# StanfordASL/GuSTO.jl

Measured on AMD Instinct MI355X. Metric: converged trajectories/sec (batched SCP), freeflyer_se2 N=50, inputs resident in HBM, higher is better.
Workload: dtype f64

## Files before the change

### gusto.jl_amd/csrc/common.hpp

```cpp
#pragma once
#include <hip/hip_runtime.h>
#include <math.h>
#include <stdint.h>

#include "gusto_hip.h"

namespace gusto {

#define GD __device__ __forceinline__
typedef double v4d __attribute__((ext_vector_type(4)));

constexpr int ROW_HARD = 0;
constexpr int ROW_PEN = 1;
constexpr int ROW_PEN_TR = 2;
constexpr int ROW_PEN_EQ = 3;
constexpr int ROW_HARD_EQ = 4;
constexpr int ROW_EQ = 5;
GD bool row_is_hard(int kind) { return kind == ROW_HARD || kind == ROW_HARD_EQ; }

constexpr int RS_T = 0, RS_LAM = 1, RS_LAMB = 2, RS_S = 3, RS_DT = 4, RS_DL = 5, RS_DS = 6, RS_KA = 7, RS_KB = 8,
              RS_NVAR = 9;

#ifndef GUSTO_DUBINS_WAVES
#define GUSTO_DUBINS_WAVES 2
#endif
#ifndef GUSTO_WAVES_PER_EU
#define GUSTO_WAVES_PER_EU 1
#endif

#ifndef GUSTO_TO_SWEEP_CALL
#define GUSTO_TO_SWEEP_CALL true
#endif
#ifndef GUSTO_TO4_SWEEP_CALL
#define GUSTO_TO4_SWEEP_CALL true
#endif
#ifndef GUSTO_SWEEP_DPP
#define GUSTO_SWEEP_DPP 1
#endif
#ifndef GUSTO_FACTOR_LDS
#define GUSTO_FACTOR_LDS 1
#endif
#ifndef GUSTO_FACTOR_LDS_MV
#define GUSTO_FACTOR_LDS_MV 1
#endif
#ifndef GUSTO_FACTOR_LDS_HUU
#define GUSTO_FACTOR_LDS_HUU 0
#endif
#ifndef GUSTO_FACTOR_LDS_ROWS
#define GUSTO_FACTOR_LDS_ROWS 1
#endif
#ifndef GUSTO_USE_MFMA
#define GUSTO_USE_MFMA true
#endif
constexpr int GUSTO_TO_FREEFLYER_SE2 = 4, GUSTO_TO_ASTROBEE_SE3 = 5, GUSTO_TO_ASTROBEE_SE3_MANIFOLD = 6;
constexpr double TRAJOPT_DEFECT_REG = 1e-4;
constexpr int RS_EARLIER = 0, RS_ROW = 1, RS_ROW_LANE = 2;
template <int MODEL> struct MT;
template <> struct MT<GUSTO_FREEFLYER_SE2> {
    static constexpr int NDEF = 0;
    static constexpr int n = 6, m = 3, WS = 2, NFIX = 3, NHU = 2;
    static constexpr int WAVES_PER_EU = GUSTO_WAVES_PER_EU;
    static constexpr int RS_FORM = RS_ROW;
    static constexpr bool SWEEP_CALL = false;
    static constexpr bool SWEEP_DPP = GUSTO_SWEEP_DPP;
    static constexpr bool FACTOR_LDS = GUSTO_FACTOR_LDS;
    static constexpr bool MFMA = false;
    static constexpr int SCHED_PROBE = 2;
    static constexpr int SCHED_SLICE = 4;
    static constexpr bool LTI = true, HAS_OBS = true;
    static constexpr bool PG2 = true;
    static constexpr int pg_r0(int c) { return c < 3 ? c : (c < 6 ? c - 3 : c - 6); }
    static constexpr int pg_r1(int c) { return c < 3 ? c + 3 : (c < 6 ? c : c - 3); }
    static constexpr bool Anz(int i, int j) { return j == i + 3; }
    static constexpr bool Mnz(int i, int j) { return i == j || j == i + 3; }
    static constexpr bool Bnz(int i, int j) { return i == j + 3; }
    static constexpr bool Gnz(int i, int j) { return i == j || i == j + 3; }
    static constexpr bool Hnz(int, int) { return true; }
};
template <> struct MT<GUSTO_DUBINS_CAR> {
    static constexpr int NDEF = 0;
    static constexpr int n = 3, m = 1, WS = 2, NFIX = 6, NHU = 2;
    static constexpr int WAVES_PER_EU = GUSTO_DUBINS_WAVES;
    static constexpr int RS_FORM = RS_ROW;
    static constexpr bool SWEEP_CALL = false;
    static constexpr bool SWEEP_DPP = false;
    static constexpr bool FACTOR_LDS = false;
    static constexpr bool MFMA = false;
    static constexpr int SCHED_PROBE = 1; static constexpr int SCHED_SLICE = 0;
    static constexpr bool LTI = false, HAS_OBS = false;
    static constexpr bool PG2 = false;
    static constexpr int pg_r0(int) { return 0; }
    static constexpr int pg_r1(int) { return 0; }
    static constexpr bool Anz(int, int) { return true; }
    static constexpr bool Mnz(int, int) { return true; }
    static constexpr bool Bnz(int, int) { return true; }
    static constexpr bool Gnz(int, int) { return true; }
    static constexpr bool Hnz(int, int) { return true; }
};
template <> struct MT<GUSTO_ASTROBEE_SE3> {
    static constexpr int NDEF = 0;
    static constexpr int n = 12, m = 6, WS = 3, NFIX = 3, NHU = 2;
    static constexpr int WAVES_PER_EU = 1;
    static constexpr int RS_FORM = RS_ROW_LANE;
    static constexpr bool SWEEP_CALL = true;
    static constexpr bool SWEEP_DPP = false;
    static constexpr bool FACTOR_LDS = false;
    static constexpr bool MFMA = GUSTO_USE_MFMA;
    static constexpr int SCHED_PROBE = 1; static constexpr int SCHED_SLICE = 0;
    static constexpr bool LTI = false, HAS_OBS = true;
    static constexpr bool PG2 = false;
    static constexpr int pg_r0(int) { return 0; }
    static constexpr int pg_r1(int) { return 0; }
    static constexpr bool Anz(int i, int j) { return i < 3 ? j == i + 3 : (i < 6 ? false : (i < 9 ? j >= 6 : j >= 9)); }
    static constexpr bool Mnz(int i, int j) { return i < 3 ? (j == i || j == i + 3) : (i < 6 ? j == i : (i < 9 ? j >= 6 : j >= 9)); }
    static constexpr bool Bnz(int i, int j) { return j < 3 ? i == j + 3 : i == j + 6; }
    static constexpr bool Gnz(int i, int j) { return j < 3 ? (i == j || i == j + 3) : i >= 6; }
    static constexpr bool Hnz(int i, int j) { return i / 3 == j / 3; }
};
template <> struct MT<GUSTO_ASTROBEE_SE3_MANIFOLD> {
    static constexpr int NDEF = 0;
    static constexpr int n = 13, m = 6, WS = 3, NFIX = 5, NHU = 2;
    static constexpr int WAVES_PER_EU = 1;
    static constexpr int RS_FORM = RS_EARLIER;
    static constexpr bool SWEEP_CALL = true ;
    static constexpr bool SWEEP_DPP = false;
    static constexpr bool FACTOR_LDS = false;
    static constexpr bool MFMA = GUSTO_USE_MFMA;
    static constexpr int SCHED_PROBE = 1; static constexpr int SCHED_SLICE = 0;
    static constexpr bool LTI = false, HAS_OBS = true;
    static constexpr bool PG2 = false;
    static constexpr int pg_r0(int) { return 0; }
    static constexpr int pg_r1(int) { return 0; }
    static constexpr bool Anz(int i, int j) { return i < 3 ? j == i + 3 : (i < 6 ? false : (i < 10 ? j >= 6 : j >= 10)); }
    static constexpr bool Mnz(int i, int j) { return i < 3 ? (j == i || j == i + 3) : (i < 6 ? j == i : (i < 10 ? j >= 6 : j >= 10)); }
    static constexpr bool Bnz(int i, int j) { return j < 3 ? i == j + 3 : i == j + 7; }
    static constexpr bool Gnz(int i, int j) { return j < 3 ? (i == j || i == j + 3) : i >= 6; }
    static constexpr int hblk(int i) { return i < 3 ? 0 : (i < 6 ? 1 : (i < 10 ? 2 : 3)); }
    static constexpr bool Hnz(int i, int j) { return hblk(i) == hblk(j); }
};

template <> struct MT<GUSTO_TO_FREEFLYER_SE2> {
    using G = MT<GUSTO_FREEFLYER_SE2>;
    static constexpr int NDEF = 6, n = 6, m = 3 + NDEF, WS = 2, NFIX = 3, NHU = 2 + 2 * NDEF;
    static constexpr int WAVES_PER_EU = 1, SCHED_PROBE = 0, SCHED_SLICE = 0;
    static constexpr int RS_FORM = RS_ROW;
    static constexpr bool SWEEP_DPP = false;
    static constexpr bool FACTOR_LDS = false;
    static constexpr bool SWEEP_CALL = GUSTO_TO4_SWEEP_CALL, MFMA = false, LTI = false, HAS_OBS = true, PG2 = false;
    static constexpr int pg_r0(int) { return 0; }
    static constexpr int pg_r1(int) { return 0; }
    static constexpr bool Anz(int i, int j) { return G::Anz(i, j); }
    static constexpr bool Mnz(int i, int j) { return G::Mnz(i, j); }
    static constexpr bool Bnz(int i, int j) { return j < G::m && G::Bnz(i, j); }
    static constexpr bool Gnz(int i, int j) { return j < G::m ? G::Gnz(i, j) : i == j - G::m; }
    static constexpr bool Hnz(int, int) { return true; }
};
template <> struct MT<GUSTO_TO_ASTROBEE_SE3> {
    using G = MT<GUSTO_ASTROBEE_SE3>;
    static constexpr int NDEF = 12, n = 12, m = 6 + NDEF, WS = 3, NFIX = 3, NHU = 2 + 2 * NDEF;
    static constexpr int WAVES_PER_EU = 1, SCHED_PROBE = 0, SCHED_SLICE = 0;
    static constexpr int RS_FORM = RS_ROW;
    static constexpr bool SWEEP_DPP = false;
    static constexpr bool FACTOR_LDS = false;
    static constexpr bool SWEEP_CALL = GUSTO_TO_SWEEP_CALL, MFMA = false, LTI = false, HAS_OBS = true, PG2 = false;
    static constexpr int pg_r0(int) { return 0; }
    static constexpr int pg_r1(int) { return 0; }
    static constexpr bool Anz(int i, int j) { return G::Anz(i, j); }
    static constexpr bool Mnz(int i, int j) { return G::Mnz(i, j); }
    static constexpr bool Bnz(int i, int j) { return j < G::m && G::Bnz(i, j); }
    static constexpr bool Gnz(int i, int j) { return j < G::m ? G::Gnz(i, j) : i == j - G::m; }
    static constexpr bool Hnz(int, int) { return true; }
};

template <> struct MT<GUSTO_TO_ASTROBEE_SE3_MANIFOLD> {
    using G = MT<GUSTO_ASTROBEE_SE3_MANIFOLD>;
    static constexpr int NDEF = 13, n = 13, m = 6 + NDEF, WS = 3, NFIX = 5, NHU = 2 + 2 * NDEF;
    static constexpr int WAVES_PER_EU = 1, SCHED_PROBE = 0, SCHED_SLICE = 0;
    static constexpr int RS_FORM = RS_ROW;
    static constexpr bool SWEEP_DPP = false;
    static constexpr bool FACTOR_LDS = false;
    static constexpr bool SWEEP_CALL = GUSTO_TO_SWEEP_CALL, MFMA = false, LTI = false, HAS_OBS = true, PG2 = false;
    static constexpr int pg_r0(int) { return 0; }
    static constexpr int pg_r1(int) { return 0; }
    static constexpr bool Anz(int i, int j) { return G::Anz(i, j); }
    static constexpr bool Mnz(int i, int j) { return G::Mnz(i, j); }
    static constexpr bool Bnz(int i, int j) { return j < G::m && G::Bnz(i, j); }
    static constexpr bool Gnz(int i, int j) { return j < G::m ? G::Gnz(i, j) : i == j - G::m; }
    static constexpr bool Hnz(int, int) { return true; }
};
constexpr double TRAJOPT_EQ_DELTA = 1e-8;

inline void warm_defaults(int model, gusto_ipm_opts& io) {
    if (io.mu_floor < 0) io.mu_floor = (model == GUSTO_ASTROBEE_SE3_MANIFOLD) ? 1e-10 : 1e-11;
    if (io.sigma_max < 0) io.sigma_max = (model == GUSTO_TO_FREEFLYER_SE2 || model == GUSTO_TO_ASTROBEE_SE3 || model == GUSTO_TO_ASTROBEE_SE3_MANIFOLD) ? 0.0 : 0.1;
    if (!(io.mu_warm < 0)) { if (io.mu_warm_gain < 0) io.mu_warm_gain = 0.0; return; }
    switch (model) {
    case GUSTO_DUBINS_CAR: io.mu_warm = 1e-9; io.mu_warm_gain = 0.0; io.mu_warm_max = 1e-9; break;
    case GUSTO_FREEFLYER_SE2: io.mu_warm = 1e-4; io.mu_warm_gain = 0.1; io.mu_warm_max = 1e-2; break;
    case GUSTO_ASTROBEE_SE3: io.mu_warm = 1e-6; io.mu_warm_gain = 1.0; io.mu_warm_max = 1e-2; break;
    default: io.mu_warm = 1e-4; io.mu_warm_gain = 1.0; io.mu_warm_max = 1e-2; break;
    }
}
constexpr double IPM_DIVERGED = 1e3;
GD double warm_mu(const gusto_ipm_opts& io, double c) {
    if (io.mu_warm == 0.0) return 0.0;
    return fmin(fmax(io.mu_warm, io.mu_warm_max), fmax(io.mu_warm, io.mu_warm_gain * c * c));
}

GD constexpr int sidx(int i, int j, int n) {
    return i <= j ? i * n - i * (i - 1) / 2 + (j - i) : j * n - j * (j - 1) / 2 + (i - j);
}

template <int MODEL> struct Rec {
    using T = MT<MODEL>;
    static constexpr int n = T::n, m = T::m, NZ = n + m;
    static constexpr int r64(int c) { return (c + 63) / 64 * 64; }
    static constexpr bool S_TRI = false;
    static constexpr int NS = S_TRI ? m * (m + 1) / 2 : m * m;
    static constexpr int SQQ = r64(NZ * (NZ + 1) / 2), SNN = r64(n * n + 1), SKD = r64(2 * m * n + NS + 1);
    static constexpr int oK = 0, oD = m * n, oS = 2 * m * n;
    static constexpr int KD_DUMMY = 2 * m * n + NS;
    static constexpr int sS(int i, int l) {
        if (!S_TRI) return oS + i * m + l;
        const int a = i < l ? i : l, b = i < l ? l : i;
        return oS + a * m - a * (a - 1) / 2 + (b - a);
    }
};

template <int MODEL> struct SpPG {
    using T = MT<MODEL>;
    static constexpr int n = T::n, m = T::m;
    static constexpr int pos_phi(int l, int i) {
        int c = 0;
// ... 384 lines not shown
GD double rcp_nr(double d) {
    double r = __builtin_amdgcn_rcp(d);
    double e = fma(-d, r, 1.0);
    r = fma(r, e, r);
    e = fma(-d, r, 1.0);
    r = fma(r, e, r);
    return r;
}

GD double rsqrt_nr(double d) {
    double r = __builtin_amdgcn_rsq(d);
    const double h = 0.5 * d;
    r = r * (1.5 - h * r * r);
    r = r * (1.5 - h * r * r);
    return r;
}

template <int m> GD bool chol_inv(const double* S, double* Li) {
    double L[m][m], r[m];
    bool ok = true;
#pragma unroll
    for (int i = 0; i < m; i++)
#pragma unroll
        for (int j = 0; j < m; j++) { L[i][j] = 0; Li[i * m + j] = 0; }
#pragma unroll
    for (int j = 0; j < m; j++) {
        double d = S[j * m + j];
#pragma unroll
        for (int l = 0; l < j; l++) d -= L[j][l] * L[j][l];
        if (!(d > 0.0)) ok = false;
        r[j] = rsqrt_nr(d);
        L[j][j] = d * r[j];
#pragma unroll
        for (int i = j + 1; i < m; i++) {
            double s = S[i * m + j];
#pragma unroll
            for (int l = 0; l < j; l++) s -= L[i][l] * L[j][l];
            L[i][j] = s * r[j];
        }
    }
#pragma unroll
    for (int j = 0; j < m; j++) {
        Li[j * m + j] = r[j];
#pragma unroll
        for (int i = j + 1; i < m; i++) {
            double s = 0;
#pragma unroll
            for (int l = j; l < i; l++) s -= L[i][l] * Li[l * m + j];
            Li[i * m + j] = s * r[i];
        }
    }
    return ok;
}

GD bool inv_spd_rt(const double* S, double* Sinv, double* Lw, int n) {
    bool ok = true;
    for (int i = 0; i < n * n; i++) { Lw[i] = 0; Sinv[i] = 0; }
    for (int j = 0; j < n; j++) {
        double d = S[j * n + j];
        for (int l = 0; l < j; l++) d -= Lw[j * n + l] * Lw[j * n + l];
        if (!(d > 0.0)) ok = false;
        d = sqrt(d);
        Lw[j * n + j] = d;
        for (int i = j + 1; i < n; i++) {
            double s = S[i * n + j];
            for (int l = 0; l < j; l++) s -= Lw[i * n + l] * Lw[j * n + l];
            Lw[i * n + j] = s / d;
        }
    }
    for (int j = 0; j < n; j++) {
        Sinv[j * n + j] = 1.0 / Lw[j * n + j];
        for (int i = j + 1; i < n; i++) {
            double s = 0;
            for (int l = j; l < i; l++) s -= Lw[i * n + l] * Sinv[l * n + j];
            Sinv[i * n + j] = s / Lw[i * n + i];
        }
    }
    for (int i = 0; i < n; i++)
        for (int j = 0; j < n; j++) {
            double s = 0;
            for (int l = (i > j ? i : j); l < n; l++) s += Sinv[l * n + i] * Sinv[l * n + j];
            Lw[i * n + j] = s;
        }
    for (int i = 0; i < n * n; i++) Sinv[i] = Lw[i];
    return ok;
}

}
```

### gusto.jl_amd/csrc/factor1w.hpp

```cpp
#pragma once

namespace gusto {


template <int MODEL, class BLK> GD double* pg_buf(const BLK& K, int k) {
    using T = MT<MODEL>;
    using R = Rec<MODEL>;
    constexpr int NPG = T::n * (T::n + T::m);
    if constexpr (LdsC<MODEL, true>::PG_LDS) return K.pgl + k * NPG;
    else if constexpr (T::LTI) return K.sPG + (k == 0 ? 2 * NPG : 0);
    else return K.sPG + (k & 1) * NPG;
}

template <int MODEL> GD void factor_sweep_1w(SweepView<MODEL> K, double* fail, Prof& pf) {
    using T = MT<MODEL>;
    using R = Rec<MODEL>;
    using C = LdsC<MODEL, true>;
    constexpr int n = T::n, m = T::m, NZ = n + m, NQ = NZ * (NZ + 1) / 2, NPG = n * NZ, NN = n * n, NZN = NZ * n;
    constexpr int RT = (NPG + 63) / 64, RQ = (NQ + 63) / 64, RN = (NN + 63) / 64, RZ = (NZN + 63) / 64, RKD = R::SKD / 64;
    const int tid = K.tid, N = K.N;
    int zJ[RZ], zG[RZ], hI[RQ], hJ[RQ], nI[RN], nJ[RN], tL[RT], tC[RT];
#pragma unroll
    for (int r = 0; r < RT; r++) { const int e = tid + 64 * r; tL[r] = (e < NPG) ? e / NZ : 0; tC[r] = (e < NPG) ? e % NZ : 0; }
#pragma unroll
// ... 359 lines not shown
                if (tid == 0) {
#pragma unroll
                    for (int e = 0; e < m * (m + 1) / 2; e++) K.kdl[k * C::KDS + 2 * m * n + e] = sp[e];
                }
            } else {
                double sv[RKD];
#pragma unroll
                for (int r = 0; r < RKD; r++) sv[r] = 0;
#pragma unroll
                for (int a = 0; a < m; a++)
#pragma unroll
                    for (int c = 0; c <= a; c++) {
                        double s = 0;
#pragma unroll
                        for (int l = a; l < m; l++) s += Li[l * m + a] * Li[l * m + c];
#pragma unroll
                        for (int r = 0; r < RKD; r++) {
                            if (64 * r + 63 < R::oS || 64 * r >= R::oS + m * m) continue;
                            const int e = tid + 64 * r - R::oS;
                            sv[r] = (e == a * m + c || e == c * m + a) ? s : sv[r];
                        }
                    }
#pragma unroll
                for (int r = 0; r < RKD; r++) {
                    const int e = tid + 64 * r;
                    double v = (r < RN) ? kdv[r < RN ? r : 0] : 0.0;
                    if (64 * r + 63 >= R::oS && 64 * r < R::oS + m * m) { if (e >= R::oS) v = sv[r]; }
                    K.KD[(size_t)k * R::SKD + e] = v;
                }
            }
        }
        if (!T::LTI && !C::PG_LDS && k > 0) {
#pragma unroll
            for (int r = 0; r < RT; r++) { const int e = tid + 64 * r; if (e < NPG) K.sPG[((k - 1) & 1) * NPG + e] = pgn[r]; }
        }
        pf.tick(PF_F7);
        K.sync();
        pf.tick(PF_FCD);
    }
}

template <int MODEL> GD void factor_sweep_pg2(SweepView<MODEL> K, double* fail, Prof& pf) {
    using T = MT<MODEL>;
    using R = Rec<MODEL>;
    using C = LdsC<MODEL, true>;
    constexpr int n = T::n, m = T::m, NZ = n + m, NQ = NZ * (NZ + 1) / 2, NPG = n * NZ, NN = n * n, NZN = NZ * n, h3 = n / 2,
                  NH = n * (n + 1) / 2;
    static_assert(T::PG2 && T::LTI && C::KD_LDS && NQ <= 64 && NZN <= 64 && NN <= 64 && n >= 2 * m, "shape");
    static_assert(T::pg_r1(0) == T::pg_r0(0) + h3 && T::pg_r1(n) == T::pg_r0(n) + h3 && T::pg_r1(n - 1) == T::pg_r0(n - 1) + h3, "PG2 row pairs");
    static_assert(NH + NN < R::SNN && !C::BIG, "P | Pi record, dummy slot");
    constexpr bool F_MV = T::FACTOR_LDS && GUSTO_FACTOR_LDS_MV, F_HUU = T::FACTOR_LDS && GUSTO_FACTOR_LDS_HUU,
                   F_ROWS = T::FACTOR_LDS && GUSTO_FACTOR_LDS_ROWS;
    static_assert(!(F_MV || F_HUU || F_ROWS) || (n == 6 && m == 3), "FACTOR_LDS: rows of three 128-bit reads, m = 2 + 1");
    constexpr bool PG_UPPER = [] { for (int c = 0; c < NZ; c++) if (!(T::pg_r0(c) < h3 && T::pg_r1(c) == T::pg_r0(c) + h3)) return false; return true; }();
    static_assert(!F_MV || PG_UPPER, "F_MV: pg_r0(c) < n/2 and pg_r1(c) = pg_r0(c) + n/2 for every column of [Phi Gam]");
    const int tid = K.tid, N = K.N;
    const int ijh = K.lut[tid < NQ ? tid : 0], hc = ijh >> 8, hj = ijh & 255, i0 = T::pg_r0(hc), j0 = T::pg_r0(hj);
    const int zc = tid < NZN ? tid / n : 0, zg = tid < NZN ? tid % n : 0, z0 = T::pg_r0(zc);
    const int ri = tid < n ? tid : 0;
    const bool isnu = tid >= 8 && tid < 8 + n;
    const bool on = tid < NN;
    const int i = on ? tid / n : 0, j = on ? tid % n : 0;
    const LPtr<double> L = K.lds;
    typedef double v2d __attribute__((ext_vector_type(2)));
    auto ld2 = [&](int off) { return *(const __attribute__((address_space(3))) v2d*)(L.p + off); };
    const int dmy = C::sT0 + (tid & 15);
    static_assert(n * NZ >= 16 + 36, "dummy slot");
    constexpr int oHuu = C::sT0 + 46, NHU = m * (m + 1) / 2;
    static_assert(oHuu % 2 == 0 && 15 + (2 * m - 1) * n < 46 && 15 + NHU < 46 && 46 + NHU <= n * NZ, "H_uu behind the dummy slots, in the T buffer");
    constexpr int NZH = F_ROWS ? NZ + 1 : NZ, oZu = (C::sZ + 1) & ~1;
    static_assert(!F_ROWS || (C::sHh % 2 == 0 && NZH % 2 == 0 && n * NZH <= NZ * NZ && oZu + 4 * n <= C::sZ + NZN), "128-bit rows of H_yu and Z_u");
    auto pcol = [](int j_) { return 2 * (j_ % h3) + j_ / h3; };
    static_assert(C::sP % 2 == 0 && C::sPi % 2 == 0 && n % 2 == 0 && C::vecs % 2 == 0, "16-byte aligned rows");
    const int oPP = C::sP + i0 * n + 2 * j0, oPZ = C::sPi + zg * n + (F_MV ? 2 * z0 : z0), oPr = C::sP + ri * n, oPir = C::sPi + ri * n;
    const int oRow = tid < n ? C::sP + tid * n : (isnu ? C::sPi + (tid - 8) * n : C::sP);
    const int wH1 = tid < NQ ? ((hc >= n && F_HUU) ? oHuu + sidx(hc - n, hj - n, m) : ((hc >= n && F_ROWS) ? dmy : C::sHh + hc * NZH + hj))
                             : dmy;
    const int wZ = tid < NZN ? (F_ROWS ? (zc >= n ? oZu + zg * 4 + (zc - n) : dmy) : C::sZ + tid) : dmy;
    const int oHi = C::sHh + i * NZH + n, oHj = C::sHh + j * NZH + n, oPn = C::sHh + (i < j ? i : j) * NZH + (i < j ? j : i);
    const int oZi = F_ROWS ? oZu + i * 4 : C::sZ + n * n + i, oZj = F_ROWS ? oZu + j * 4 : C::sZ + n * n + j;
    const int wP = on ? C::sP + i * n + pcol(j) : dmy, wPi = on ? C::sPi + j * n + (F_MV ? pcol(i) : i) : dmy, wGd = on ? C::sGd + tid : dmy;
    const int vecs = C::vecs, oCv = vecs + 3 * N * n, oRv = vecs + 4 * N * n, oNun = vecs + 6 * N * n;
    const int wRv = tid < n ? oRv + tid : dmy, wNun = tid < n ? oNun + tid : dmy, sRv = tid < n ? n : 0;
    const int wRN = tid < n ? oRv + tid : (isnu ? oNun + (tid - 8) : dmy), sRN = (tid < n || isnu) ? n : 0;
    const int kdo = K.kd_off;
    const int wKD = tid < n ? kdo + tid : dmy, sKD = tid < n ? C::KDS : 0;
    const int wSi = tid == 0 ? kdo + 2 * m * n : dmy, sSi = tid == 0 ? C::KDS : 0;
    const int ep = (on && i <= j) ? sidx(i, j, n) : R::SNN - 1, eq = on ? NH + tid : R::SNN - 1;
    struct PGC { double a0, a1, b0, b1, zv0, zv1; };
    double Bd[n * m];
    Dyn<MODEL>::B(*K.mpp, Bd);
    auto pg_main = [&](int r_, int c_) { return K.PGk(N - 1)[r_ * NZ + c_]; };
    auto pg_zero = [&](int r_, int c_) {
        double v = 0.0;
#pragma unroll
        for (int q = 0; q < n * m; q++) if (c_ >= n && q == r_ * m + (c_ - n)) v = 0.5 * K.dt * Bd[q];
        return v;
    };
    PGC cN, c0;
    cN.a0 = pg_main(i0, hc); cN.a1 = pg_main(i0 + h3, hc); cN.b0 = pg_main(j0, hj); cN.b1 = pg_main(j0 + h3, hj);
    cN.zv0 = pg_main(z0, zc); cN.zv1 = pg_main(z0 + h3, zc);
    c0.a0 = pg_zero(i0, hc); c0.a1 = pg_zero(i0 + h3, hc); c0.b0 = pg_zero(j0, hj); c0.b1 = pg_zero(j0 + h3, hj);
    c0.zv0 = pg_zero(z0, zc); c0.zv1 = pg_zero(z0 + h3, zc);
    const double eterm = pg_main(zg, zc) + ((zc == zg) ? 1.0 : 0.0);
    const bool egoal = K.is_goal(zg);
    L[wP] = 0.0; L[wPi] = 0.0; L[wZ] = 0.0;
    double gdR = 0.0, zR = 0.0;
    if (tid < R::SNN) K.Paft[(size_t)(N - 1) * R::SNN + tid] = 0.0;
    double qq = K.kdl[(N - 1) * C::KDS + (tid < NQ ? tid : 0)];
    double LiP[m * m], wiP[m];
#pragma unroll
    for (int e = 0; e < m * m; e++) LiP[e] = 0.0;
#pragma unroll
    for (int e = 0; e < m; e++) wiP[e] = 0.0;
    bool okall = true;
    K.sync();

    auto tail = [&](int kt, const double* zi, const double* zj) {
        double pin = zR, gd = gdR;
        double vi[m], vj[m], dj[m];
#pragma unroll
        for (int a = 0; a < m; a++) {
            double s3 = 0, s4 = 0;
#pragma unroll
            for (int l = 0; l <= a; l++) { s3 += LiP[a * m + l] * zi[l]; s4 += LiP[a * m + l] * zj[l]; }
            vi[a] = s3; vj[a] = s4;
        }
#pragma unroll
        for (int a = 0; a < m; a++) {
            double s2 = 0;
#pragma unroll
            for (int l = a; l < m; l++) s2 += LiP[l * m + a] * vj[l];
            dj[a] = s2;
        }
#pragma unroll
        for (int l = 0; l < m; l++) { pin -= wiP[l] * vj[l]; gd += vi[l] * vj[l]; }
        L[wPi] = pin; gdR = gd;
        K.Paft[(size_t)(kt - 1) * R::SNN + eq] = pin;
#pragma unroll
        for (int a = 0; a < m; a++) L[wKD + kt * sKD + (m + a) * n] = dj[a];
    };

    auto msync = [&]() {
#ifdef GUSTO_STRICT_SYNC
        asm volatile("s_waitcnt vmcnt(0) lgkmcnt(0)\n\ts_barrier" ::: "memory");
#endif
        __builtin_amdgcn_fence(__ATOMIC_ACQ_REL, "wavefront");
    };
#if defined(GUSTO_PROFILE) && defined(GUSTO_STAGE_PROF)
#define STAMP(v) const unsigned long long v = __builtin_amdgcn_s_memtime()
#define STAMPS_END() do { pf.acc[PF_FPRE] += (long long)(t1_ - t0_); pf.acc[PF_FAB] += (long long)(t2_ - t1_); \
                          pf.acc[PF_F4] += (long long)(t3_ - t2_); pf.acc[PF_F5] += (long long)(t4_ - t3_); pf.acc[PF_FCD] += (long long)(t5_ - t4_); } while (0)
#else
#define STAMP(v) do {} while (0)
#define STAMPS_END() do {} while (0)
#endif
    auto ld3 = [&](int oi, int oj, double* vi, double* vj) {
        const v2d a2 = ld2(oi), b2 = ld2(oj);
        vi[0] = a2.x; vi[1] = a2.y; vi[2] = L[oi + 2]; vj[0] = b2.x; vj[1] = b2.y; vj[2] = L[oj + 2];
    };
    auto stage = [&](int k, const PGC& c, bool last) {
        STAMP(t0_);
        const v2d pA = ld2(oPP), pB = ld2(oPP + h3 * n);
        const double p00 = pA.x, p01 = pA.y, p10 = pB.x, p11 = pB.y;
        double ra[n], rb[n];
        if constexpr (!F_MV) {
#pragma unroll
            for (int l = 0; l < n; l += 2) {
                const v2d a2 = ld2(oPr + l), b2 = ld2(oCv + k * n + l);
                ra[l / 2] = a2.x; ra[l / 2 + h3] = a2.y; rb[l] = b2.x; rb[l + 1] = b2.y;
            }
        }
        double zi[m], zj[m];
        if constexpr (F_ROWS) ld3(oZi, oZj, zi, zj);
        else {
#pragma unroll
            for (int l = 0; l < m; l++) { zi[l] = L[oZi + l * n]; zj[l] = L[oZj + l * n]; }
        }
        const double qqn = K.kdl[((k > 0) ? k - 1 : 0) * C::KDS + (tid < NQ ? tid : 0)];
        const double h = qq + c.a0 * (c.b0 * p00 + c.b1 * p01) + c.a1 * (c.b0 * p10 + c.b1 * p11);
        L[wH1] = h;
        if constexpr (!F_MV) {
            double rr = 0;
#pragma unroll
            for (int l = 0; l < n; l++) rr += ra[l] * rb[l];
            L[wRv + k * sRv] = rr;
        }
        STAMP(t1_);
        msync();
        double S[m * m], Li[m * m];
        if constexpr (F_HUU) {
            const v2d s0 = ld2(oHuu), s1 = ld2(oHuu + 2), s2 = ld2(oHuu + 4);
            const double su[NHU] = {s0.x, s0.y, s1.x, s1.y, s2.x, s2.y};
#pragma unroll
            for (int a = 0; a < m; a++)
#pragma unroll
                for (int b = 0; b < m; b++) S[a * m + b] = su[sidx(a, b, m)];
        } else {
#pragma unroll
            for (int a = 0; a < m; a++)
#pragma unroll
                for (int b = 0; b < m; b++) {
                    const int e = sidx(n + (a < b ? a : b), n + (a < b ? b : a), NZ);
                    S[a * m + b] = readlane_f64(h, e);
                }
        }
        double hi[m], hjv[m];
        if constexpr (F_ROWS) ld3(oHi, oHj, hi, hjv);
        else {
#pragma unroll
            for (int l = 0; l < m; l++) { hi[l] = L[oHi + l]; hjv[l] = L[oHj + l]; }
        }
        double pn = L[oPn];
        tail(k + 1 < N ? k + 1 : N - 1, zi, zj);
        STAMP(t2_);
        msync();
        const double zb0 = F_MV ? ld2(oPZ).x : L[oPZ], zb1 = F_MV ? ld2(oPZ).y : L[oPZ + h3];
        double pa[n];
#pragma unroll
        for (int l = 0; l < n; l += 2) {
            const v2d a2 = ld2((F_MV ? oRow : oPir) + l);
            if constexpr (F_MV) {
                const v2d b2 = ld2(oCv + k * n + l);
                pa[l / 2] = a2.x; pa[l / 2 + h3] = a2.y; rb[l] = b2.x; rb[l + 1] = b2.y;
            } else { pa[l] = a2.x; pa[l + 1] = a2.y; }
        }
        okall = chol_inv<m>(S, Li) && okall;
        STAMP(t3_);
        {
            double z = c.zv0 * zb0 + c.zv1 * zb1;
            const double zE = fma(0.5, eterm, z);
            z = (last && egoal) ? zE : z;
            L[wZ] = z;
            zR = z;
            double rr = 0;
#pragma unroll
            for (int l = 0; l < n; l++) rr += pa[l] * rb[l];
            if constexpr (F_MV) L[wRN + k * sRN] = rr;
            else L[wNun + k * sRv] = rr;
        }
        STAMP(t4_);
        double wi[m], wj[m], kj[m];
#pragma unroll
        for (int a = 0; a < m; a++) {
            double s1 = 0, s2 = 0;
#pragma unroll
            for (int l = 0; l <= a; l++) { s1 += Li[a * m + l] * hi[l]; s2 += Li[a * m + l] * hjv[l]; }
            wi[a] = s1; wj[a] = s2;
        }
#pragma unroll
        for (int a = 0; a < m; a++) {
            double s1 = 0;
#pragma unroll
            for (int l = a; l < m; l++) s1 += Li[l * m + a] * wj[l];
            kj[a] = s1;
        }
#pragma unroll
        for (int l = 0; l < m; l++) pn -= wi[l] * wj[l];
        L[wP] = pn;
        K.Paft[(size_t)(k - 1) * R::SNN + ep] = pn;
#pragma unroll
        for (int a = 0; a < m; a++) L[wKD + k * sKD + a * n] = kj[a];
        {
#pragma unroll
            for (int a = 0; a < m; a++)
#pragma unroll
                for (int b = 0; b <= a; b++) {
                    double s1 = 0;
#pragma unroll
                    for (int l = a; l < m; l++) s1 += Li[l * m + a] * Li[l * m + b];
                    L[wSi + k * sSi + sidx(b, a, m)] = s1;
                }
        }
        qq = qqn;
#pragma unroll
        for (int e = 0; e < m * m; e++) LiP[e] = Li[e];
#pragma unroll
        for (int e = 0; e < m; e++) wiP[e] = wi[e];
        msync();
        STAMP(t5_);
        STAMPS_END();
    };
#undef STAMP
#undef STAMPS_END

    for (int k = N - 1; k >= 1; k--) stage(k, cN, k == N - 1);
    stage(0, c0, false);
    {
        double zi[m], zj[m];
        if constexpr (F_ROWS) ld3(oZi, oZj, zi, zj);
        else {
#pragma unroll
            for (int l = 0; l < m; l++) { zi[l] = L[oZi + l * n]; zj[l] = L[oZj + l * n]; }
        }
        tail(0, zi, zj);
    }
    L[wGd] = gdR;
    if (!okall) *fail = 1.0;
    K.sync();
    (void)pf;
}

#ifndef GUSTO_COSTATE_ADJOINT
#define GUSTO_COSTATE_ADJOINT 1
#endif
template <int MODEL> constexpr bool costate_adjoint() { return GUSTO_COSTATE_ADJOINT && MT<MODEL>::SWEEP_CALL && MT<MODEL>::MFMA; }
#ifndef GUSTO_ADJ_MAX_IT
#define GUSTO_ADJ_MAX_IT 20
#endif
#ifndef GUSTO_ADJ_ACC
#define GUSTO_ADJ_ACC 3
#endif
constexpr int ADJ_FLAG = 9;
template <int MODEL> GD bool costate_adjoint_now() { return gusto_dyn_lds[LdsC<MODEL, true>::misc + ADJ_FLAG] != 0.0; }
template <int MODEL> GD bool costate_adjoint_rt(const gusto_model_params& mp, double dt) {
    if constexpr (MODEL == GUSTO_ASTROBEE_SE3) return 0.5 * dt * mp.hard_limit_omega <= 0.65;
    else return true;
}
template <int MODEL, bool NOPP, bool SEG = false>
GD void factor_sweep_mfma(SweepView<MODEL> K, double* fail, Prof& pf, int kHi_ = 0, int kLo_ = 0, bool isA = false, int oP = 0, int oPi = 0,
                          int oGd = -1) {
    using T = MT<MODEL>;
    using R = Rec<MODEL>;
    constexpr int n = T::n, m = T::m, NZ = n + m, NPG = n * NZ, NN = n * n;
    using SP = SpPG<MODEL>;
    constexpr bool SPR = SP::USE;
    constexpr int KS = (n + 3) / 4, MS = (m + 3) / 4, RT = SPR ? (SP::NS + 63) / 64 : (NPG + 63) / 64, RN = (NN + 63) / 64;
    static_assert(!T::LTI && n <= 15 && m <= 8 && R::SNN > NN && R::SKD > 2 * m * n + m * m, "tile / record shape");
#ifdef GUSTO_PROFILE_COARSE
#define FT_(id) do { } while (0)
#else
#define FT_(id) pf.tick(id)
#endif
    const int tid = K.tid, N = K.N;
    const int kHi = SEG ? kHi_ : N - 1, kLo = SEG ? kLo_ : 0;
    const int mi = tid & 15, mq = tid >> 4;
    constexpr bool adj_rt = NOPP;
// ... 252 lines not shown
```

### gusto.jl_amd/csrc/ipm.hpp

```cpp
#pragma once
#include "rows.hpp"

#ifndef GUSTO_COOP_CHOL_MIN
#define GUSTO_COOP_CHOL_MIN 7
#endif

namespace gusto {

extern __shared__ __attribute__((aligned(16))) double gusto_dyn_lds[];

template <int MODEL> constexpr bool costate_adjoint();

struct IpmOut {
    int status, iters;
    double obj, res_p, res_d, mu;
};

template <bool ONEWAVE> GD void blk_sync() {
    if constexpr (ONEWAVE) {
#ifdef GUSTO_STRICT_SYNC
        asm volatile("s_waitcnt vmcnt(0) lgkmcnt(0)\n\ts_barrier" ::: "memory");
#endif
        __builtin_amdgcn_fence(__ATOMIC_ACQ_REL, "wavefront");
        __builtin_amdgcn_wave_barrier();
// ... 1627 lines not shown
            double acc = 0;
#pragma unroll
            for (int l = 0; l < n; l++) acc += Li[l * n + i] * Li[l * n + j];
            if (e < n * n) K.sP[e] = acc;
        }
        return;
    }
    for (int e = tid; e < n * n; e += nt) {
        const int i = e / n, j = e % n;
        if (i == j && !K.is_goal(i)) A[e] = 1.0;
        Li[e] = 0.0;
    }
    K.sync();
    for (int j = 0; j < n; j++) {
        const double ajj = A[j * n + j];
        if (!(ajj > 0.0)) *fail = 1.0;
        const double d = rsqrt_nr(ajj);
        K.sync();
        if (tid >= j && tid < n) A[tid * n + j] *= d;
        K.sync();
        for (int e = tid; e < n * n; e += nt) {
            const int i = e / n, c = e % n;
            if (c > j && i >= c) A[e] -= A[i * n + j] * A[c * n + j];
        }
        K.sync();
    }
    if (tid < n) {
        const int c = tid;
        Li[c * n + c] = rcp_nr(A[c * n + c]);
        for (int i = c + 1; i < n; i++) {
            double acc = 0;
            for (int l = c; l < i; l++) acc -= A[i * n + l] * Li[l * n + c];
            Li[i * n + c] = acc * rcp_nr(A[i * n + i]);
        }
    }
    K.sync();
    for (int e = tid; e < n * n; e += nt) {
        const int i = e / n, j = e % n;
        double acc = 0;
        for (int l = (i > j ? i : j); l < n; l++) acc += Li[l * n + i] * Li[l * n + j];
        K.sP[e] = acc;
    }
}

template <int MODEL, class BLK, int NCH = 0> GD void mid_phase(BLK& K, int k, bool act, double hdt, double* red, double* mugn, Prof* pf = nullptr) {
    constexpr bool SEG = NCH > 0;
#define MT_(i) do { if (pf) pf->tick(i); } while (0)
    MT_(PF_MID);
    using T = MT<MODEL>;
    using R = Rec<MODEL>;
    constexpr int n = T::n, m = T::m, NZ = n + m;
    const int N = K.N;
    double th[n], d0[m];
    constexpr bool KEEP_D = T::SWEEP_CALL && BLK::ONE && !BLK::C::KD_LDS;
    double Dk[KEEP_D ? m * n : 1];
#pragma unroll
    for (int i = 0; i < (KEEP_D ? m * n : 1); i++) Dk[i] = 0;
#pragma unroll
    for (int i = 0; i < n; i++) th[i] = 0;
#pragma unroll
    for (int i = 0; i < m; i++) d0[i] = 0;
    if (act) {
        double tt[n], lu[m], Gamk[n * m];
        constexpr bool GT_RECOMP = !T::LTI && n > 8 && T::NDEF == 0;
        double gterm[n], gsub[n];
        if (k >= 1) {
            if constexpr (T::PG2 || (!T::LTI && n > 8 && T::NDEF == 0)) {
                double Mk_[n * n];
                load_M_Gam(K, k, Mk_, Gamk);
                if constexpr (GT_RECOMP) {
#pragma unroll
                    for (int j = 0; j < n; j++) {
                        double g = 0.0;
#pragma unroll
                        for (int i = 0; i < n; i++) if (T::Mnz(j, i)) g += Mk_[j * n + i] * K.rd_(k, i);
                        gterm[j] = g; gsub[j] = K.misc[64 + j] - K.Xw[k * n + j];
                    }
                }
            } else {
                const auto pg = K.PGk(k);
#pragma unroll
                for (int i = 0; i < n; i++)
#pragma unroll
                    for (int j = 0; j < m; j++) Gamk[i * m + j] = T::Gnz(i, j) ? pg[i * NZ + n + j] : 0.0;
            }
        } else {
            Dyn<MODEL>::B(K.P.mp, Gamk);
#pragma unroll
            for (int i = 0; i < n * m; i++) Gamk[i] *= hdt;
            if constexpr (T::NDEF > 0) {
#pragma unroll
                for (int i = 0; i < T::NDEF; i++) Gamk[i * m + (m - T::NDEF) + i] = 1.0;
            }
        }
#pragma unroll
        for (int i = 0; i < n; i++) tt[i] = K.pv[k * n + i];
#pragma unroll
        for (int i = 0; i < m; i++) {
            double s = K.qu_(k, i);
#pragma unroll
            for (int l = 0; l < n; l++) if (T::Gnz(l, i)) s += Gamk[l * m + i] * tt[l];
            lu[i] = s;
        }
#pragma unroll
        for (int i = 0; i < m; i++) {
            double s = 0;
#pragma unroll
            for (int l = 0; l < m; l++) s += K.kdS(k, i, l) * lu[l];
            d0[i] = s;
        }
        if constexpr (T::LTI) {
            double rdl[n], Mg[n * n];
            if constexpr (T::PG2) {
                double Gg[n * m];
                load_M_Gam(K, k, Mg, Gg);
            } else {
                const auto pg = K.PGk(0);
#pragma unroll
                for (int j = 0; j < n; j++)
#pragma unroll
                    for (int i = 0; i < n; i++) Mg[j * n + i] = T::Mnz(j, i) ? 0.5 * (pg[j * NZ + i] + (i == j ? 1.0 : 0.0)) : 0.0;
            }
#pragma unroll
            for (int i = 0; i < n; i++) rdl[i] = K.rd_(k, i);
#pragma unroll
            for (int j = 0; j < n; j++) {
                double g = 0.0;
#pragma unroll
                for (int i = 0; i < n; i++) if (T::Mnz(j, i)) g += Mg[j * n + i] * rdl[i];
                gterm[j] = g; gsub[j] = K.misc[64 + j] - K.Xw[k * n + j];
            }
        }
        double thd[n];
#pragma unroll
        for (int j = 0; j < n; j++) thd[j] = K.nun[k * n + j];
#pragma unroll
        for (int i = 0; i < m; i++)
#pragma unroll
            for (int j = 0; j < n; j++) {
                const double dij = K.kd(k, R::oD + i * n + j);
                if constexpr (KEEP_D) Dk[i * n + j] = dij;
                thd[j] -= dij * lu[i];
            }
#pragma unroll
        for (int j = 0; j < n; j++) {
            double s = thd[j];
            if constexpr (T::LTI || GT_RECOMP) {
                s = (k == N - 1 && K.is_goal(j)) ? (s + gterm[j]) - gsub[j] : s;
            } else
            if (k == N - 1 && K.is_goal(j)) {
                const auto pg = K.PGk(k);
#pragma unroll
                for (int i = 0; i < n; i++) s += 0.5 * (pg[j * NZ + i] + (i == j ? 1.0 : 0.0)) * K.rd_(k, i);
                s -= K.misc[64 + j] - K.Xw[k * n + j];
            }
            th[j] = s;
        }
    }
    MT_(PF_M_TH);
    if constexpr (SEG) {
        using SB = SegB<MODEL, NCH>;
        constexpr int NI = NCH - 1;
        const LPtr<double> L = K.lds;
        const int sb = K.P.ll.seg;
        const int ri = K.tid < n ? K.tid : 0;
        double r[NCH * n];
        {
            constexpr int MAXL = (64 + NCH - 1) / NCH + 1;
            const int tb = sb + SB::sPG2(0);
            if (act) {
#pragma unroll
                for (int j = 0; j < n; j++) L[tb + k * n + j] = th[j];
            }
            K.sync();
            const int t = K.tid < NCH * n ? K.tid : NCH * n - 1, tc = t / n, tj = t % n;
            const int k0 = seg_lo(tc, N, NCH), k1 = seg_lo(tc + 1, N, NCH);
            double v[MAXL];
#pragma unroll
            for (int q = 0; q < MAXL; q++) v[q] = L[tb + ((k0 + q < k1) ? k0 + q : k0) * n + tj];
            __builtin_amdgcn_sched_barrier(0);
            double s = 0;
#pragma unroll
            for (int q = 0; q < MAXL; q++) s += (k0 + q < k1) ? v[q] : 0.0;
#pragma unroll
            for (int e = 0; e < NCH * n; e++) r[e] = readlane_f64(s, e);
        }
        MT_(PF_M_RED);
        auto row = [&](int o, double* v) {
#pragma unroll
            for (int l = 0; l < n; l++) v[l] = L[o + ri * n + l];
        };
        auto col = [&](int o, double* v) {
#pragma unroll
            for (int l = 0; l < n; l++) v[l] = L[o + l * n + ri];
// ... 942 lines not shown
```

Before: 149,500.

## Store Cholesky inverse factor and defer S^-1 and D formation to the solve

In the freeflyer factor sweep, the per-stage S^-1 = L^-T L^-1 products and the D = L^-T v back-substitution are no longer formed in the serial backward factorization. Instead, the stored L^-1 and v are written, and the forward/solve kernel reconstructs S^-1 and D in registers when it needs them. This shortens the latency-bound sequential factor loop at the cost of extra arithmetic and register pressure in the more parallel solve phase. An optional DPP row-broadcast path for H_uu is also added but disabled by default.

```diff
diff --git a/gusto.jl_amd/csrc/common.hpp b/gusto.jl_amd/csrc/common.hpp
--- a/gusto.jl_amd/csrc/common.hpp
+++ b/gusto.jl_amd/csrc/common.hpp
@@ -49,6 +49,17 @@
 #ifndef GUSTO_FACTOR_LDS_ROWS
 #define GUSTO_FACTOR_LDS_ROWS 1
 #endif
+#ifndef GUSTO_FACTOR_HUU_DPP
+#define GUSTO_FACTOR_HUU_DPP 0
+#endif
+#ifndef GUSTO_FACTOR_LAZY_SINV
+#define GUSTO_FACTOR_LAZY_SINV 1
+#endif
+#ifndef GUSTO_FACTOR_LAZY_D
+#define GUSTO_FACTOR_LAZY_D 1
+#endif
+static_assert(!(GUSTO_FACTOR_LDS_HUU && GUSTO_FACTOR_HUU_DPP), "H_uu to the Cholesky through LDS or by DPP, not both");
+static_assert(!GUSTO_FACTOR_LAZY_D || GUSTO_FACTOR_LAZY_SINV, "GUSTO_FACTOR_LAZY_D forms D from the L^-1 that GUSTO_FACTOR_LAZY_SINV stores");
 #ifndef GUSTO_USE_MFMA
 #define GUSTO_USE_MFMA true
 #endif
@@ -64,6 +75,7 @@
     static constexpr bool SWEEP_CALL = false;
     static constexpr bool SWEEP_DPP = GUSTO_SWEEP_DPP;
     static constexpr bool FACTOR_LDS = GUSTO_FACTOR_LDS;
+    static constexpr bool FACTOR_REC = true;
     static constexpr bool MFMA = false;
     static constexpr int SCHED_PROBE = 2;
     static constexpr int SCHED_SLICE = 4;
@@ -85,6 +97,7 @@
     static constexpr bool SWEEP_CALL = false;
     static constexpr bool SWEEP_DPP = false;
     static constexpr bool FACTOR_LDS = false;
+    static constexpr bool FACTOR_REC = false;
     static constexpr bool MFMA = false;
     static constexpr int SCHED_PROBE = 1; static constexpr int SCHED_SLICE = 0;
     static constexpr bool LTI = false, HAS_OBS = false;
@@ -105,6 +118,7 @@
     static constexpr bool SWEEP_CALL = true;
     static constexpr bool SWEEP_DPP = false;
     static constexpr bool FACTOR_LDS = false;
+    static constexpr bool FACTOR_REC = false;
     static constexpr bool MFMA = GUSTO_USE_MFMA;
     static constexpr int SCHED_PROBE = 1; static constexpr int SCHED_SLICE = 0;
     static constexpr bool LTI = false, HAS_OBS = true;
@@ -125,6 +139,7 @@
     static constexpr bool SWEEP_CALL = true ;
     static constexpr bool SWEEP_DPP = false;
     static constexpr bool FACTOR_LDS = false;
+    static constexpr bool FACTOR_REC = false;
     static constexpr bool MFMA = GUSTO_USE_MFMA;
     static constexpr int SCHED_PROBE = 1; static constexpr int SCHED_SLICE = 0;
     static constexpr bool LTI = false, HAS_OBS = true;
@@ -146,6 +161,7 @@
     static constexpr int RS_FORM = RS_ROW;
     static constexpr bool SWEEP_DPP = false;
     static constexpr bool FACTOR_LDS = false;
+    static constexpr bool FACTOR_REC = false;
     static constexpr bool SWEEP_CALL = GUSTO_TO4_SWEEP_CALL, MFMA = false, LTI = false, HAS_OBS = true, PG2 = false;
     static constexpr int pg_r0(int) { return 0; }
     static constexpr int pg_r1(int) { return 0; }
@@ -162,6 +178,7 @@
     static constexpr int RS_FORM = RS_ROW;
     static constexpr bool SWEEP_DPP = false;
     static constexpr bool FACTOR_LDS = false;
+    static constexpr bool FACTOR_REC = false;
     static constexpr bool SWEEP_CALL = GUSTO_TO_SWEEP_CALL, MFMA = false, LTI = false, HAS_OBS = true, PG2 = false;
     static constexpr int pg_r0(int) { return 0; }
     static constexpr int pg_r1(int) { return 0; }
@@ -179,6 +196,7 @@
     static constexpr int RS_FORM = RS_ROW;
     static constexpr bool SWEEP_DPP = false;
     static constexpr bool FACTOR_LDS = false;
+    static constexpr bool FACTOR_REC = false;
     static constexpr bool SWEEP_CALL = GUSTO_TO_SWEEP_CALL, MFMA = false, LTI = false, HAS_OBS = true, PG2 = false;
     static constexpr int pg_r0(int) { return 0; }
     static constexpr int pg_r1(int) { return 0; }
@@ -669,6 +687,31 @@
     }
     return ok;
 }
+template <int m> GD double sinv_entry(const double* Li, int a, int b) {
+    double s1 = 0;
+#pragma unroll
+    for (int l = a; l < m; l++) s1 += Li[l * m + a] * Li[l * m + b];
+    return s1;
+}
+template <int m> GD double lt_entry(const double* Li, const double* v, int a) {
+    double s2 = 0;
+#pragma unroll
+    for (int l = a; l < m; l++) s2 += Li[l * m + a] * v[l];
+    return s2;
+}
+template <int Q> GD double row_bcast_f64(double v) {
+    const unsigned long long u = __builtin_bit_cast(unsigned long long, v);
+    const int lo = (int)(u & 0xffffffffu), hi = (int)(u >> 32);
+    const unsigned rl = (unsigned)__builtin_amdgcn_update_dpp(0, lo, 0x150 + Q, 0xf, 0xf, true);
+    const unsigned rh = (unsigned)__builtin_amdgcn_update_dpp(0, hi, 0x150 + Q, 0xf, 0xf, true);
+    return __builtin_bit_cast(double, ((unsigned long long)rh << 32) | rl);
+}
+GD void row_bcast6_b64(double v, double* s) {
+    asm("s_nop 1\n\tv_mov_b64_dpp %0, %6 row_newbcast:0 row_mask:0xf bank_mask:0xf\n\tv_mov_b64_dpp %1, %6 row_newbcast:1 row_mask:0xf bank_mask:0xf\n\t"
+        "v_mov_b64_dpp %2, %6 row_newbcast:2 row_mask:0xf bank_mask:0xf\n\tv_mov_b64_dpp %3, %6 row_newbcast:3 row_mask:0xf bank_mask:0xf\n\t"
+        "v_mov_b64_dpp %4, %6 row_newbcast:4 row_mask:0xf bank_mask:0xf\n\tv_mov_b64_dpp %5, %6 row_newbcast:5 row_mask:0xf bank_mask:0xf"
+        : "=&v"(s[0]), "=&v"(s[1]), "=&v"(s[2]), "=&v"(s[3]), "=&v"(s[4]), "=&v"(s[5]) : "v"(v));
+}
 
 GD bool inv_spd_rt(const double* S, double* Sinv, double* Lw, int n) {
     bool ok = true;
diff --git a/gusto.jl_amd/csrc/factor1w.hpp b/gusto.jl_amd/csrc/factor1w.hpp
--- a/gusto.jl_amd/csrc/factor1w.hpp
+++ b/gusto.jl_amd/csrc/factor1w.hpp
@@ -435,10 +435,21 @@
     constexpr bool F_MV = T::FACTOR_LDS && GUSTO_FACTOR_LDS_MV, F_HUU = T::FACTOR_LDS && GUSTO_FACTOR_LDS_HUU,
                    F_ROWS = T::FACTOR_LDS && GUSTO_FACTOR_LDS_ROWS;
     static_assert(!(F_MV || F_HUU || F_ROWS) || (n == 6 && m == 3), "FACTOR_LDS: rows of three 128-bit reads, m = 2 + 1");
+    constexpr bool F_DPP = T::FACTOR_REC && GUSTO_FACTOR_HUU_DPP, F_LSINV = T::FACTOR_REC && GUSTO_FACTOR_LAZY_SINV,
+                   F_LD = T::FACTOR_REC && GUSTO_FACTOR_LAZY_D;
+    constexpr int NHU = m * (m + 1) / 2, NHY = NQ - NHU;
+    static_assert(!(F_DPP && F_HUU) && (!F_LD || F_LSINV), "H_uu by DPP or through LDS; D from the stored L^-1");
+    constexpr auto hmap = [](int t) { const int row = t >> 4, pos = t & 15, e = (16 - NHU) * row + pos - NHU; return pos < NHU ? NHY + pos : (e < NHY ? e : -1); };
+    static_assert(!F_DPP || (NHU == 6 && sidx(n, n, NZ) == NHY && 4 * (16 - NHU) >= NHY), "H_uu is the tail of the packed H; four rows hold the rest");
+    constexpr bool HMAP_ONCE = [&] { for (int e = 0; e < NHY; e++) { int c = 0; for (int t = 0; t < 64; t++) c += hmap(t) == e; if (c != 1) return false; } return true; }();
+    constexpr bool HMAP_HUU = [&] { for (int t = 0; t < 64; t++) if ((t & 15) < NHU ? hmap(t) != NHY + (t & 15) : hmap(t) >= NHY) return false; return true; }();
+    static_assert(!F_DPP || HMAP_ONCE, "every entry of rows 0 .. n-1 of H is formed by exactly one lane");
+    static_assert(!F_DPP || HMAP_HUU, "the upper triangle of H_uu sits at positions 0 .. 5 of each of the four rows of lanes, and nowhere else");
     constexpr bool PG_UPPER = [] { for (int c = 0; c < NZ; c++) if (!(T::pg_r0(c) < h3 && T::pg_r1(c) == T::pg_r0(c) + h3)) return false; return true; }();
     static_assert(!F_MV || PG_UPPER, "F_MV: pg_r0(c) < n/2 and pg_r1(c) = pg_r0(c) + n/2 for every column of [Phi Gam]");
     const int tid = K.tid, N = K.N;
-    const int ijh = K.lut[tid < NQ ? tid : 0], hc = ijh >> 8, hj = ijh & 255, i0 = T::pg_r0(hc), j0 = T::pg_r0(hj);
+#define HEQ_ (F_DPP ? (hmap(tid) >= 0 ? hmap(tid) : 0) : (tid < NQ ? tid : 0))
+    const int ijh = K.lut[HEQ_], hc = ijh >> 8, hj = ijh & 255, i0 = T::pg_r0(hc), j0 = T::pg_r0(hj);
     const int zc = tid < NZN ? tid / n : 0, zg = tid < NZN ? tid % n : 0, z0 = T::pg_r0(zc);
     const int ri = tid < n ? tid : 0;
     const bool isnu = tid >= 8 && tid < 8 + n;
@@ -449,7 +460,7 @@
     auto ld2 = [&](int off) { return *(const __attribute__((address_space(3))) v2d*)(L.p + off); };
     const int dmy = C::sT0 + (tid & 15);
     static_assert(n * NZ >= 16 + 36, "dummy slot");
-    constexpr int oHuu = C::sT0 + 46, NHU = m * (m + 1) / 2;
+    constexpr int oHuu = C::sT0 + 46;
     static_assert(oHuu % 2 == 0 && 15 + (2 * m - 1) * n < 46 && 15 + NHU < 46 && 46 + NHU <= n * NZ, "H_uu behind the dummy slots, in the T buffer");
     constexpr int NZH = F_ROWS ? NZ + 1 : NZ, oZu = (C::sZ + 1) & ~1;
     static_assert(!F_ROWS || (C::sHh % 2 == 0 && NZH % 2 == 0 && n * NZH <= NZ * NZ && oZu + 4 * n <= C::sZ + NZN), "128-bit rows of H_yu and Z_u");
@@ -457,7 +468,7 @@
     static_assert(C::sP % 2 == 0 && C::sPi % 2 == 0 && n % 2 == 0 && C::vecs % 2 == 0, "16-byte aligned rows");
     const int oPP = C::sP + i0 * n + 2 * j0, oPZ = C::sPi + zg * n + (F_MV ? 2 * z0 : z0), oPr = C::sP + ri * n, oPir = C::sPi + ri * n;
     const int oRow = tid < n ? C::sP + tid * n : (isnu ? C::sPi + (tid - 8) * n : C::sP);
-    const int wH1 = tid < NQ ? ((hc >= n && F_HUU) ? oHuu + sidx(hc - n, hj - n, m) : ((hc >= n && F_ROWS) ? dmy : C::sHh + hc * NZH + hj))
+    const int wH1 = (F_DPP ? hmap(tid) >= 0 : tid < NQ) ? ((hc >= n && F_HUU) ? oHuu + sidx(hc - n, hj - n, m) : ((hc >= n && F_ROWS) ? dmy : C::sHh + hc * NZH + hj))
                              : dmy;
     const int wZ = tid < NZN ? (F_ROWS ? (zc >= n ? oZu + zg * 4 + (zc - n) : dmy) : C::sZ + tid) : dmy;
     const int oHi = C::sHh + i * NZH + n, oHj = C::sHh + j * NZH + n, oPn = C::sHh + (i < j ? i : j) * NZH + (i < j ? j : i);
@@ -490,7 +501,7 @@
     L[wP] = 0.0; L[wPi] = 0.0; L[wZ] = 0.0;
     double gdR = 0.0, zR = 0.0;
     if (tid < R::SNN) K.Paft[(size_t)(N - 1) * R::SNN + tid] = 0.0;
-    double qq = K.kdl[(N - 1) * C::KDS + (tid < NQ ? tid : 0)];
+    double qq = K.kdl[(N - 1) * C::KDS + HEQ_];
     double LiP[m * m], wiP[m];
 #pragma unroll
     for (int e = 0; e < m * m; e++) LiP[e] = 0.0;
@@ -509,19 +520,16 @@
             for (int l = 0; l <= a; l++) { s3 += LiP[a * m + l] * zi[l]; s4 += LiP[a * m + l] * zj[l]; }
             vi[a] = s3; vj[a] = s4;
         }
-#pragma unroll
-        for (int a = 0; a < m; a++) {
-            double s2 = 0;
-#pragma unroll
-            for (int l = a; l < m; l++) s2 += LiP[l * m + a] * vj[l];
-            dj[a] = s2;
+        if constexpr (!F_LD) {
+#pragma unroll
+            for (int a = 0; a < m; a++) dj[a] = lt_entry<m>(LiP, vj, a);
         }
 #pragma unroll
         for (int l = 0; l < m; l++) { pin -= wiP[l] * vj[l]; gd += vi[l] * vj[l]; }
         L[wPi] = pin; gdR = gd;
         K.Paft[(size_t)(kt - 1) * R::SNN + eq] = pin;
 #pragma unroll
-        for (int a = 0; a < m; a++) L[wKD + kt * sKD + (m + a) * n] = dj[a];
+        for (int a = 0; a < m; a++) L[wKD + kt * sKD + (m + a) * n] = F_LD ? vj[a] : dj[a];
     };
 
     auto msync = [&]() {
@@ -560,7 +568,7 @@
 #pragma unroll
             for (int l = 0; l < m; l++) { zi[l] = L[oZi + l * n]; zj[l] = L[oZj + l * n]; }
         }
-        const double qqn = K.kdl[((k > 0) ? k - 1 : 0) * C::KDS + (tid < NQ ? tid : 0)];
+        const double qqn = K.kdl[((k > 0) ? k - 1 : 0) * C::KDS + HEQ_];
         const double h = qq + c.a0 * (c.b0 * p00 + c.b1 * p01) + c.a1 * (c.b0 * p10 + c.b1 * p11);
         L[wH1] = h;
         if constexpr (!F_MV) {
@@ -575,6 +583,17 @@
         if constexpr (F_HUU) {
             const v2d s0 = ld2(oHuu), s1 = ld2(oHuu + 2), s2 = ld2(oHuu + 4);
             const double su[NHU] = {s0.x, s0.y, s1.x, s1.y, s2.x, s2.y};
+#pragma unroll
+            for (int a = 0; a < m; a++)
+#pragma unroll
+                for (int b = 0; b < m; b++) S[a * m + b] = su[sidx(a, b, m)];
+        } else if constexpr (F_DPP) {
+            double su[NHU];
+            if constexpr (GUSTO_FACTOR_HUU_DPP == 2) row_bcast6_b64(h, su);
+            else {
+                su[0] = row_bcast_f64<0>(h); su[1] = row_bcast_f64<1>(h); su[2] = row_bcast_f64<2>(h);
+                su[3] = row_bcast_f64<3>(h); su[4] = row_bcast_f64<4>(h); su[5] = row_bcast_f64<5>(h);
+            }
 #pragma unroll
             for (int a = 0; a < m; a++)
 #pragma unroll
@@ -644,16 +663,16 @@
         K.Paft[(size_t)(k - 1) * R::SNN + ep] = pn;
 #pragma unroll
         for (int a = 0; a < m; a++) L[wKD + k * sKD + a * n] = kj[a];
-        {
+        if constexpr (F_LSINV) {
 #pragma unroll
             for (int a = 0; a < m; a++)
 #pragma unroll
-                for (int b = 0; b <= a; b++) {
-                    double s1 = 0;
-#pragma unroll
-                    for (int l = a; l < m; l++) s1 += Li[l * m + a] * Li[l * m + b];
-                    L[wSi + k * sSi + sidx(b, a, m)] = s1;
-                }
+                for (int b = 0; b <= a; b++) L[wSi + k * sSi + sidx(b, a, m)] = Li[a * m + b];
+        } else {
+#pragma unroll
+            for (int a = 0; a < m; a++)
+#pragma unroll
+                for (int b = 0; b <= a; b++) L[wSi + k * sSi + sidx(b, a, m)] = sinv_entry<m>(Li, a, b);
         }
         qq = qqn;
 #pragma unroll
@@ -666,6 +685,7 @@
     };
 #undef STAMP
 #undef STAMPS_END
+#undef HEQ_
 
     for (int k = N - 1; k >= 1; k--) stage(k, cN, k == N - 1);
     stage(0, c0, false);
diff --git a/gusto.jl_amd/csrc/ipm.hpp b/gusto.jl_amd/csrc/ipm.hpp
--- a/gusto.jl_amd/csrc/ipm.hpp
+++ b/gusto.jl_amd/csrc/ipm.hpp
@@ -1703,7 +1703,9 @@
     constexpr int n = T::n, m = T::m, NZ = n + m;
     const int N = K.N;
     double th[n], d0[m];
-    constexpr bool KEEP_D = T::SWEEP_CALL && BLK::ONE && !BLK::C::KD_LDS;
+    constexpr bool REC = T::FACTOR_REC && BLK::ONE && BLK::C::KD_LDS && !SEG, REC_SINV = REC && GUSTO_FACTOR_LAZY_SINV, REC_D = REC && GUSTO_FACTOR_LAZY_D;
+    static_assert(!REC || (T::PG2 && !T::SWEEP_CALL && !T::MFMA), "FACTOR_REC: the kernel whose factor sweep is factor_sweep_pg2");
+    constexpr bool KEEP_D = (T::SWEEP_CALL && BLK::ONE && !BLK::C::KD_LDS) || REC_D;
     double Dk[KEEP_D ? m * n : 1];
 #pragma unroll
     for (int i = 0; i < (KEEP_D ? m * n : 1); i++) Dk[i] = 0;
@@ -1753,12 +1755,37 @@
             for (int l = 0; l < n; l++) if (T::Gnz(l, i)) s += Gamk[l * m + i] * tt[l];
             lu[i] = s;
         }
+        double Lk[REC_SINV ? m * m : 1], Sk[REC_SINV ? m * (m + 1) / 2 : 1];
+        if constexpr (REC_SINV) {
+#pragma unroll
+            for (int a = 0; a < m; a++)
+#pragma unroll
+                for (int b = 0; b < m; b++) Lk[a * m + b] = (b <= a) ? K.kdl[k * BLK::C::KDS + 2 * m * n + sidx(b, a, m)] : 0.0;
+#pragma unroll
+            for (int a = 0; a < m; a++)
+#pragma unroll
+                for (int b = 0; b <= a; b++) Sk[sidx(b, a, m)] = sinv_entry<m>(Lk, a, b);
+        }
 #pragma unroll
         for (int i = 0; i < m; i++) {
             double s = 0;
 #pragma unroll
-            for (int l = 0; l < m; l++) s += K.kdS(k, i, l) * lu[l];
+            for (int l = 0; l < m; l++) {
+                double sil;
+                if constexpr (REC_SINV) sil = Sk[sidx(i, l, m)]; else sil = K.kdS(k, i, l);
+                s += sil * lu[l];
+            }
             d0[i] = s;
+        }
+        if constexpr (REC_D) {
+#pragma unroll
+            for (int j = 0; j < n; j++) {
+                double vj[m];
+#pragma unroll
+                for (int l = 0; l < m; l++) vj[l] = K.kd(k, R::oD + l * n + j);
+#pragma unroll
+                for (int a = 0; a < m; a++) Dk[a * n + j] = lt_entry<m>(Lk, vj, a);
+            }
         }
         if constexpr (T::LTI) {
             double rdl[n], Mg[n * n];
@@ -1789,8 +1816,12 @@
         for (int i = 0; i < m; i++)
 #pragma unroll
             for (int j = 0; j < n; j++) {
-                const double dij = K.kd(k, R::oD + i * n + j);
-                if constexpr (KEEP_D) Dk[i * n + j] = dij;
+                double dij;
+                if constexpr (REC_D) dij = Dk[i * n + j];
+                else {
+                    dij = K.kd(k, R::oD + i * n + j);
+                    if constexpr (KEEP_D) Dk[i * n + j] = dij;
+                }
                 thd[j] -= dij * lu[i];
             }
 #pragma unroll
```

New measurement: 152,700 (median of 6 runs). 1.02x the previous value.
